# bdaiinstitute/judo

Measured on AMD Instinct MI355X. Metric: rollouts/sec + plan-step ms, leap_cube MPPI 65536xH64, higher is better.
Workload: dtype f32

## Files before the change

### judo_amd/csrc/jh_api.hip

```cpp
#include <algorithm>
#include <cmath>
#include <cstdlib>
#include <cstring>

#include "jh_internal.h"
#include "jh_update_dev.h"

static thread_local char g_err[512] = "";

void jh_set_error(const char* fmt, ...) {
  va_list ap;
  va_start(ap, fmt);
  vsnprintf(g_err, sizeof(g_err), fmt, ap);
  va_end(ap);
}

extern "C" const char* jh_last_error(void) { return g_err; }
extern "C" int jh_version(void) { return 100; }

static int image_cylinders(const jh_blob_header& h, const float* F, const int* I) {
  constexpr int HEADER = 24, BODY_I = 6, BODY_F = 32, BLOCK_I = 4, DOF_F = 20, ACT_I = 2, ACT_F = 8, GEOM_I = 2, GEOM_F = 20, GF_RBOUND = 15;
  if (h.nint < (uint32_t)HEADER || h.nfloat < (uint32_t)HEADER) return 0;
  const long NM = I[0], NBLK = I[1], nv = I[2], nu = I[4], NG = I[5];
  if (NM < 0 || NBLK < 0 || nv < 0 || nu < 0 || NG < 0) return 0;
// ... 279 lines not shown
  const char* e = getenv("JUDO_AMD_LATENCY_SHIFT");
  if (e && e[0] >= '0' && e[0] <= '2') return (e[0] - '0') < most ? (e[0] - '0') : most;
  const long alone = (long)cus * 4;
  for (int sh = most; sh > 0; sh--) if (((long)N << sh) <= alone * rpw) return sh;
  return 0;
}

static int max_fused_knots(const jh_model* m, int H) {
  const bool coop = m->kernel_gen >= 2 && (m->kind == JH_TASK_LEAP_CUBE || m->kind == JH_TASK_FR3_PICK);
  int k = JH_MAX_KNOT_DIM / (m->nu > 0 ? m->nu : 1);
  if (coop && m->kind == JH_TASK_LEAP_CUBE && m->kernel_gen >= 3) return k;
  if (coop) return k < 8 ? k : 8;
  const int lds_k = (m->kind == JH_TASK_CARTPOLE || m->kind == JH_TASK_CYLINDER_PUSH) ? jh_simple_max_knots(m, H) : (g_xcheck.max_knots ? g_xcheck.max_knots(m, H) : 0);
  return k < lds_k ? k : lds_k;
}

extern "C" int jh_model_limits(const jh_model* m, int* out) {
  JH_REQUIRE(m && out, "model_limits: null pointer");
  out[0] = max_fused_knots(m, 1);
  out[1] = JH_MAX_KNOT_DIM;
  out[2] = JH_MAX_ELITES;
  const jh_engine_build* eb = engine_build(m);
  out[3] = eb ? eb->contact_capacity : (articulated(m) ? 32 : 0);
  return JH_OK;
}

extern "C" int jh_model_max_fused_knots(const jh_model* m, int H) {
  JH_REQUIRE(m != nullptr && H >= 1, "model_max_fused_knots: null model or H < 1");
  return max_fused_knots(m, H);
}

extern "C" int jh_model_one_launch_max_knots(const jh_model* m, int H) {
  JH_REQUIRE(m != nullptr && H >= 1, "model_one_launch_max_knots: null model or H < 1");
  const int k = JH_MAX_KNOT_DIM / (m->nu > 0 ? m->nu : 1), lds_k = jh_simple_one_launch_max_knots(m, H);
  return k < lds_k ? k : lds_k;
}

extern "C" int jh_model_set_plan_step_launches(jh_model* m, int launches) {
  JH_REQUIRE(m != nullptr && launches >= 0 && launches <= 2, "model_set_plan_step_launches: launches must be 0 (automatic), 1 or 2");
  JH_REQUIRE(launches != 1 || m->kind == JH_TASK_CARTPOLE || m->kind == JH_TASK_CYLINDER_PUSH, "model_set_plan_step_launches: only the closed-form models have a one-launch plan step");
  m->plan_step_launches = launches;
  return JH_OK;
}

extern "C" int jh_model_set_rollout_schedule(jh_model* m, int mode) {
  JH_REQUIRE(m != nullptr && mode >= 0 && mode <= 2, "model_set_rollout_schedule: mode must be 0 (automatic), 1 (static grid) or 2 (persistent waves wherever the kernel has them)");
  m->rollout_schedule = mode;
  return JH_OK;
}

extern "C" int jh_model_set_rollout_slices(jh_model* m, int slices, int max_workgroups, int flags) {
  JH_REQUIRE(m != nullptr && slices >= 0 && slices <= 64, "model_set_rollout_slices: slices must be 0 (automatic) or 1 .. 64");
  JH_REQUIRE(max_workgroups >= 0, "model_set_rollout_slices: max_workgroups must be 0 (the resident slots) or a positive cap on the queue's grid");
  JH_REQUIRE((flags & ~1) == 0, "model_set_rollout_slices: flags has bit 0 (every hand-off counts as missed) and no other");
  m->rollout_slices = slices; m->rollout_max_workgroups = max_workgroups; m->rollout_slice_flags = flags;
  m->rollout_nbounds = 0;
  return JH_OK;
}

extern "C" int jh_model_set_rollout_slice_bounds(jh_model* m, const int* first_steps, int n) {
  JH_REQUIRE(m != nullptr && n >= 0 && n <= JH_MAX_SLICE_BOUNDS && (n == 0 || first_steps != nullptr), "model_set_rollout_slice_bounds: 0 (none) to %d first steps", JH_MAX_SLICE_BOUNDS);
  for (int i = 0; i < n; i++)
    JH_REQUIRE(first_steps[i] > (i ? first_steps[i - 1] : 0), "model_set_rollout_slice_bounds: first steps must be positive and strictly increasing (entry %d is %d)", i, first_steps[i]);
  for (int i = 0; i < n; i++) m->rollout_bounds[i] = first_steps[i];
  m->rollout_nbounds = n;
  if (n > 0) m->rollout_slices = 0;
  return JH_OK;
}

extern "C" int jh_model_last_rollout_slice_bounds(const jh_model* m, int* out, int cap) {
  JH_REQUIRE(m != nullptr && cap >= 0 && (cap == 0 || out != nullptr), "model_last_rollout_slice_bounds: null model or output");
  const int n = __atomic_load_n(&m->last_rollout_nbounds, __ATOMIC_RELAXED);
  for (int i = 0; i < n && i < cap; i++) out[i] = __atomic_load_n(&m->last_rollout_bounds[i], __ATOMIC_RELAXED);
  return n;
}

void jh_model_note_slice_bounds(const jh_model* m, int slices, int H, const int* bounds) {
  const int n = slices > 1 ? (slices - 1 < 63 ? slices - 1 : 63) : 0;
  for (int i = 0; i < n; i++) __atomic_store_n(&m->last_rollout_bounds[i], bounds ? bounds[i] : (i + 1) * H / slices, __ATOMIC_RELAXED);
  __atomic_store_n(&m->last_rollout_nbounds, n, __ATOMIC_RELAXED);
}

#ifndef JH_AUTO_TAPER
#define JH_AUTO_TAPER 1
#endif
constexpr int JH_TAPER_DEPTH = 4, JH_TAPER_MIN_H = 32;
extern "C" int jh_rollout_slice_schedule(int H, int groups, int wave_slots, int* first_steps, int cap) {
  JH_REQUIRE(H >= 0 && groups >= 0 && wave_slots >= 0 && cap >= 0 && (cap == 0 || first_steps != nullptr), "rollout_slice_schedule: negative argument or null output");
  int b[4], n = 0;
  if (wave_slots > 0 && (long long)groups >= 2ll * wave_slots) {
    if (JH_AUTO_TAPER && H >= JH_TAPER_MIN_H && (long long)groups >= (long long)JH_TAPER_DEPTH * wave_slots) {
      const long long num[4] = {6, 10, 13, 15};
      for (n = 0; n < 4; n++) b[n] = (int)(num[n] * H / 16);
    } else {
      const int S = H < 4 ? H : 4;
      for (int i = 1; i < S; i++) b[n++] = i * H / S;
    }
  }
  for (int i = 0; i < n && i < cap; i++) first_steps[i] = b[i];
  return n;
}

extern "C" int jh_model_last_rollout_slices(const jh_model* m) {
  JH_REQUIRE(m != nullptr, "model_last_rollout_slices: null model");
  return __atomic_load_n(&m->last_rollout_slices, __ATOMIC_RELAXED);
}

extern "C" int jh_model_recomputed_units(jh_model* m) {
  JH_REQUIRE(m != nullptr, "model_recomputed_units: null model");
  int v = 0;
  JH_HIP(hipMemcpy(&v, m->d_stats + JH_STAT_RECOMPUTED, sizeof(int), hipMemcpyDeviceToHost));
  return v;
}

extern "C" int jh_upload_async(void* dst, const void* src, size_t nbytes, void* stream) {
  JH_REQUIRE(dst && src, "upload_async: null pointer");
  JH_HIP(hipMemcpyAsync(dst, src, nbytes, hipMemcpyHostToDevice, (hipStream_t)stream));
  return JH_OK;
}

extern "C" int jh_download_wait(void* dst, const void* src, size_t nbytes, void* stream) {
  JH_REQUIRE(dst && src, "download_wait: null pointer");
  JH_HIP(hipMemcpyAsync(dst, src, nbytes, hipMemcpyDeviceToHost, (hipStream_t)stream));
  JH_HIP(hipStreamSynchronize((hipStream_t)stream));
  return JH_OK;
}

// ... 473 lines not shown
```

### judo_amd/csrc/jh_engine_v5.hip

```cpp
#include <cstddef>
#include <type_traits>

#include "jh_coop.h"

using namespace jh_eng;
using namespace jh_coop;

namespace {

#ifdef JH_V5_WAVESTAMP
__device__ unsigned long long* g_wavestamp = nullptr;
__device__ int g_wavestamp_cap = 0;
#endif

constexpr int G = 16, RPW = 4, WAVE = 64;
constexpr int NCH = 4, NLK = 4;

constexpr int LSMAX = 16;
constexpr int WAVES_PER_EU = 2;
constexpr int WAVES_PER_BLOCK = 4;
constexpr int BFS = 33;
constexpr int PAS = 9;
constexpr int RSPAD = 4;
constexpr int C3PAD = 278;
constexpr int NSLDS = 3;
constexpr double BIGPROB = 0.999999;
constexpr int CVX_STOP_NM = 1000;
#define OPAQUE(x) asm volatile("" : "+v"(x))
constexpr int PARK_F = 5 * 64;
struct SliceBounds { unsigned w[8]; };
constexpr int MAX_BOUND_SLICES = 16;
#define PARK_LD(p) __hip_atomic_load((p), __ATOMIC_RELAXED, __HIP_MEMORY_SCOPE_AGENT)
#define PARK_ST(p, v) __hip_atomic_store((p), (v), __ATOMIC_RELAXED, __HIP_MEMORY_SCOPE_AGENT)
#define WSYNC() do { __builtin_amdgcn_fence(__ATOMIC_RELEASE, "wavefront"); __builtin_amdgcn_wave_barrier(); __builtin_amdgcn_fence(__ATOMIC_ACQUIRE, "wavefront"); } while (0)
#ifndef JH_V5_NSLOT
#define JH_V5_NSLOT 2
#endif
#ifndef JH_V5_NSBIG
#define JH_V5_NSBIG 3
#endif
#ifndef JH_V5_CYL
#define JH_V5_CYL 0
#endif
constexpr int GCYL = 5;
constexpr int NSLOT = JH_V5_NSLOT;
constexpr int NSBIG = JH_V5_NSBIG;
constexpr int NCP = 16 * (NSBIG < NSLDS ? NSBIG : NSLDS);
constexpr int NCAP = 16 * NSBIG;
constexpr int NOVF = NCAP - NCP;
constexpr int MAXHIT = 64;
constexpr int POOL_F = 10;
constexpr int MAXG = 80, MAXLG = 8;
constexpr int CUBE = 17;
constexpr int HITPAIR = 1 << 15;
static_assert(MAXG <= 128, "hand geom pairs are packed into 14 bits");
constexpr int MAXBP = 128;
constexpr int PT_SLOT = JH_PT_SLOT, PT_MAX = JH_PT_MAX, PT_I = JH_PT_I;
constexpr int MAXBPL = 96;
constexpr int NDH = 22 * 23 / 2;
constexpr int NV = 22, NQ = 23, NU = 16, NS = 31, NS_CALTECH = 23, NX = 45, NMB = 17;
constexpr int NBC = 20;
__device__ __forceinline__ bool static_code(int b) { return b == 0 || b >= NMB; }

enum { LC_DAMP = 0, LC_KVD, LC_KP, LC_KV, LC_CLO, LC_CHI, LC_CLIM, LC_FL, LC_FB, LC_FD, LC_INVW, LC_LIMITED, LC_LO, LC_HI, LC_LK, LC_LB, LC_SI, LC_IMCK = LC_SI + 5, LC_N = 25 };

struct __attribute__((aligned(16))) RS {
  float pa[NMB][PAS];
  float xR[NMB][9];
  float qv[NV], g[NV], p[NV], ws[NV];
  float acn[6];
  float Mbb[NCH][10];
  float rhs6[6];
  float cmd[4];
  union {
    struct {
      float bs[NBC][4];
      unsigned short hits[MAXHIT];
      unsigned char bpl[MAXBPL];
    };
    struct { float pk_q[G], pk_fs[G], pk_cq[4], pk_acc; };
  };
  union {
// ... 209 lines not shown
  for (int i = 3; i >= 0; i--) { float s = x[i];
#pragma unroll
    for (int k = i + 1; k < 4; k++) s -= L[tri(k, i)] * x[k];
    x[i] = s * inv[i]; }
}
__device__ __forceinline__ float sel4(const float* a, int j) { return j == 0 ? a[0] : (j == 1 ? a[1] : (j == 2 ? a[2] : a[3])); }

__device__ __forceinline__ float sel4o(const float* a, int j) {
  float lo = (j & 1) ? a[1] : a[0], hi = (j & 1) ? a[3] : a[2];
  asm volatile("" : "+v"(lo), "+v"(hi));
  float r = (j & 2) ? hi : lo;
  asm volatile("" : "+v"(r));
  return r;
}

__device__ __forceinline__ int pidx(int a, int b) { return a * (7 - a) / 2 + (b - a - 1); }
__device__ __forceinline__ bool chain_elim_order(int cmask, int c, int& level, int& parent, int& maxlev) {
  int adj[NCH] = {0, 0, 0, 0};
#pragma unroll
  for (int a = 0; a < NCH; a++)
#pragma unroll
    for (int b = a + 1; b < NCH; b++) if ((cmask >> (4 * a + b)) & 1) { adj[a] |= 1 << b; adj[b] |= 1 << a; }
  int rem = 0xF; bool ok = true;
  level = 0; parent = -1; maxlev = 0;
#pragma unroll
  for (int st = 0; st < NCH; st++) {
    int elig = 0, pr[NCH] = {-1, -1, -1, -1};
#pragma unroll
    for (int a = 0; a < NCH; a++) if ((rem >> a) & 1) {
      const int nbm = adj[a] & rem, deg = __popc(nbm);
      if (deg == 0) elig |= 1 << a;
      else if (deg == 1) {
        const int nb = __ffs(nbm) - 1;
        const int anb = nb == 0 ? adj[0] : (nb == 1 ? adj[1] : (nb == 2 ? adj[2] : adj[3]));
        if (__popc(anb & rem) > 1 || a < nb) { elig |= 1 << a; pr[a] = nb; }
      }
    }
    if (rem != 0 && elig == 0) ok = false;
    if (elig != 0) maxlev = st;
#pragma unroll
    for (int a = 0; a < NCH; a++) if (((elig >> a) & 1) && a == c) { level = st; parent = pr[a]; }
    rem &= ~elig;
  }
  return ok;
}

template <bool MATERIALIZE, int WPB, bool SELF, bool PERSIST = false, bool BATCH = false>
__global__ __launch_bounds__(WAVE * WPB, WAVES_PER_EU) void k_leap_v5(const float* __restrict__ gF, const int* __restrict__ gI, const float* __restrict__ x0, int x0_batched,
                                                   const float* __restrict__ nominal, const float* __restrict__ noise, int ldn,
                                                   const float* __restrict__ sigma, const float* __restrict__ W, const float* __restrict__ lohi,
                                                   const float* __restrict__ tp, int N, int n_offset, int H, int K, float* __restrict__ costs,
                                                   float* __restrict__ knots_out, const float* __restrict__ controls, float* __restrict__ states,
                                                   float* __restrict__ sensors, int* __restrict__ stats_, int dshift_, float* __restrict__ trace, float* __restrict__ ovf_all_, unsigned* __restrict__ head,
                                                   long long batch_blk, long long batch_noise, long long batch_image, unsigned* pflags, int slices_, SliceBounds sb_) {
  static_assert(!BATCH || (!MATERIALIZE && !PERSIST), "batched launches are fused launches on the static grid");
  if constexpr (BATCH) {
    const long long pb = blockIdx.y;
    x0 += pb * batch_blk; nominal += pb * batch_blk; sigma += pb * batch_blk; lohi += pb * batch_blk; tp += pb * batch_blk;
    noise += pb * batch_noise; costs += pb * N; gF += pb * batch_image;
    if (trace) trace += pb * N * H * 15;
    if (NOVF > 0 && ovf_all_) ovf_all_ += pb * N * (NOVF * POOL_F);
  }
  __shared__ RS sRS[RPW * WPB];
  __shared__ float sBody[16 * BFS];
  __shared__ float sTp[16];
  __shared__ float sGeomF[MAXG * GEOM_F];
  __shared__ int sGeomI[MAXG * GEOM_I];
  __shared__ int sLaneG[16 * MAXLG];
  __shared__ float sLane[16 * LC_N];
  __shared__ int sBP[SELF ? 2 * MAXBP : 4];
  __shared__ int sBG[SELF ? 2 * NBC : 4];
  __shared__ float sBB[SELF ? NBC * 8 : 4];
  __shared__ int sGrp[WPB];
  __shared__ int sUnit[4 * WPB];
  const int dshift = PERSIST ? 0 : dshift_;
#ifdef JH_V5_WAVESTAMP
  const unsigned long long ws_entry = wall_clock64(); unsigned long long ws_staged = ws_entry;
#endif
  const int tid = threadIdx.x, wv = tid >> 6, lane = tid & 63, r = lane >> 4;
  int l = lane & 15, c = l >> 2, s = l & 3;
  RS& S = sRS[wv * RPW + r];
  const int nmI = gI[0], nblkI = gI[1], nuI = gI[4], ngI = gI[5], nsiteI = gI[6], nsI = gI[7], oRef = gI[18];
  const int oBodyF = HEADER_F, oDofF = oBodyF + nmI * BODY_F, oActF = oDofF + gI[2] * DOF_F, oGeomF = oActF + nuI * ACT_F, oSiteF = oGeomF + ngI * GEOM_F;
  const int oGeomI = HEADER_I + nmI * BODY_I + nblkI * BLOCK_I + nuI * ACT_I, oSiteI = oGeomI + ngI * GEOM_I;
  const int oLane = gI[11], lgm = gI[12];
  const int oBP = gI[15], oBS = gI[16], nBP = gI[17], oBG = oBP + 2 * nBP;
  for (int i = tid; i < 16 * BODY_F; i += WAVE * WPB) sBody[(i / BODY_F) * BFS + i % BODY_F] = gF[oBodyF + BODY_F + i];
  for (int i = tid; i < ngI * GEOM_F; i += WAVE * WPB) sGeomF[i] = gF[oGeomF + i];
  for (int i = tid; i < ngI * GEOM_I; i += WAVE * WPB) sGeomI[i] = gI[oGeomI + i];
  for (int i = tid; i < 16 * lgm; i += WAVE * WPB) sLaneG[i] = gI[oLane + i];
  if (!MATERIALIZE && tid < 9) sTp[tid] = tp[tid];
  if constexpr (SELF) {
    for (int i = tid; i < 2 * nBP && i < 2 * MAXBP; i += WAVE * WPB) sBP[i] = gI[oBP + i];
    for (int i = tid; i < 2 * NBC; i += WAVE * WPB) sBG[i] = gI[oBG + i];
    for (int i = tid; i < NBC * 8; i += WAVE * WPB) sBB[i] = gF[oBS + i];
  }
  if (tid < 16) {
    const float* df = gF + oDofF + (6 + l) * DOF_F; const float* af = gF + oActF + l * ACT_F;
    float* lc = sLane + l * LC_N;
    lc[LC_DAMP] = df[DF_DAMP]; lc[LC_KVD] = df[DF_KV]; lc[LC_FL] = df[DF_FL]; lc[LC_FB] = df[DF_FB]; lc[LC_FD] = df[DF_FD]; lc[LC_INVW] = df[DF_INVW];
    lc[LC_LIMITED] = df[DF_LIMITED]; lc[LC_LO] = df[DF_LO]; lc[LC_HI] = df[DF_HI]; lc[LC_LK] = df[DF_LK]; lc[LC_LB] = df[DF_LB];
    for (int k = 0; k < 5; k++) lc[LC_SI + k] = df[DF_SOLIMP + k];
    lc[LC_KP] = af[AF_KP]; lc[LC_KV] = af[AF_KV]; lc[LC_CLIM] = af[AF_CLIM]; lc[LC_CLO] = af[AF_CLO]; lc[LC_CHI] = af[AF_CHI];
    lc[LC_IMCK] = l < 6 ? 1.f / (l < 3 ? gF[HF_CMASS] : gF[HF_CINERTIA + (l < 3 ? 0 : l - 3)]) : 0.f;
  }
  const float* lc = sLane + l * LC_N;
  int grp = blockIdx.x * WPB + wv;
  const int ngroups = (N + RPW - 1) / RPW;
  if constexpr (PERSIST) {
    __syncthreads();
#ifdef JH_V5_WAVESTAMP
    ws_staged = wall_clock64();
#endif
  }
  int unit = grp;
  const int nsl = PERSIST ? max(1, min(slices_ & 0xff, H)) : 1, nunits = nsl * ngroups;
  float* park = (float*)(pflags + ((nunits + 3) & ~3));
  bool again = false;
  float q, qd, qc[7], vc[6], acc;
#ifdef JH_V5_WAVESTAMP
  unsigned long long ws_start = 0;
#endif
  for (; !PERSIST || unit < nunits;) {
  bool resumed = false, prefix = false; int hh0 = 0;
  if constexpr (PERSIST) if (again) {
    unit = __builtin_amdgcn_readfirstlane(sUnit[4 * wv + 3]); grp = unit % ngroups; hh0 = __builtin_amdgcn_readfirstlane(sUnit[4 * wv + 1]);
    const int h1 = __builtin_amdgcn_readfirstlane(sUnit[4 * wv + 2]);
    WSYNC();
    if (lane == 0) sUnit[4 * wv] = h1;
  }
  if constexpr (PERSIST) if (!again) {
    grp = unit % ngroups;
    const int sl = unit / ngroups; int h0 = sl * H / nsl, h1 = (sl + 1) * H / nsl;
    if (slices_ & 0x200) {
      const auto bound = [&](int i) -> int { return (int)((sb_.w[i >> 1] >> ((i & 1) << 4)) & 0xffffu); };
      h1 = bound(sl); h0 = sl > 0 ? bound(sl - 1) : 0;
    }
    if (sl > 0) {
      unsigned f = 0;
      if (lane == 0 && !(slices_ & 0x100)) f = __hip_atomic_load(pflags + (unit - ngroups), __ATOMIC_ACQUIRE, __HIP_MEMORY_SCOPE_AGENT);
      resumed = __builtin_amdgcn_readfirstlane(f) != 0;
      if (resumed) { __builtin_amdgcn_fence(__ATOMIC_ACQUIRE, "agent"); hh0 = h0; }
      prefix = !resumed;
    }
    if (lane == 0) { sGrp[wv] = grp; sUnit[4 * wv] = (sl == 0 || resumed) ? h1 : h0; sUnit[4 * wv + 1] = h0; sUnit[4 * wv + 2] = h1; sUnit[4 * wv + 3] = unit; }
  }
#ifdef JH_V5_WAVESTAMP
  if (!PERSIST || !again) ws_start = wall_clock64();
#endif
  const int n = (grp << (2 - dshift)) + (r >> dshift);
  const bool live = n < N && (r & ((1 << dshift) - 1)) == 0;
  const int nc = n < N ? n : N - 1;
  int* stats = stats_; float* ovf_all = ovf_all_;
  if constexpr (PERSIST) if (prefix) {
    stats = nullptr;
    if (NOVF > 0 && ovf_all_) ovf_all = ovf_all_ + ((long long)N + (long long)(blockIdx.x * WPB + wv) * RPW + r - nc) * (NOVF * POOL_F);
  }
  const float h = gF[HF_DT], impratio = gF[HF_IMPRATIO], tol = gF[HF_TOL], lstol = gF[HF_LSTOL]; const int cap = (int)gF[HF_MAXITER];
  const float grav[3] = {gF[HF_GRAV], gF[HF_GRAV + 1], gF[HF_GRAV + 2]};
  const float cmass = gF[HF_CMASS], cI[3] = {gF[HF_CINERTIA], gF[HF_CINERTIA + 1], gF[HF_CINERTIA + 2]};
  const float chs[3] = {gF[HF_CSIZE], gF[HF_CSIZE + 1], gF[HF_CSIZE + 2]}, crb = gF[HF_CRBOUND], ctran = gF[HF_CTRAN];
  const float cK = gF[HF_CK], cB = gF[HF_CB];
  float csi[5]; for (int k = 0; k < 5; k++) csi[k] = gF[HF_SOLIMP + k];
  const float mck = (l < 3 ? cmass : (l == 3 ? cI[0] : (l == 4 ? cI[1] : (l == 5 ? cI[2] : 0.f))));
  if (!PERSIST || !again) {
    const float* xi = x0 + ((MATERIALIZE && x0_batched) ? (size_t)nc * NX : 0);
    for (int k = 0; k < 7; k++) qc[k] = xi[k];
    for (int k = 0; k < 6; k++) vc[k] = xi[NQ + k];
    q = xi[7 + l]; qd = xi[NQ + 6 + l];
  }
  auto knot_at = [&](int k, int ll, int ncc) -> float {
    const int i = k * NU + ll;
    float v = nominal[i];
    if (n_offset + ncc != 0) v = fmaf(sigma[i], noise[(size_t)i * ldn + ncc], v);
    return jh_clampf(v, lohi[ll], lohi[NU + ll]);
  };
  if (!MATERIALIZE) {
    if (knots_out && live && (!PERSIST || unit < ngroups)) for (int k = 0; k < K; k++) knots_out[(size_t)(k * NU + l) * ldn + n] = knot_at(k, l, nc);
  }
  if (!PERSIST || !again) { S.ws[6 + l] = 0.f; if (l < 6) S.ws[l] = 0.f; }
  if (l < 4) S.cmd[l] = l == 0 ? cmass : (l == 1 ? cI[0] : (l == 2 ? cI[1] : cI[2]));
  int n_iters = 0, n_maxed = 0, n_wave_iters = 0;
  if (!PERSIST || !again) acc = 0.f;
  if constexpr (PERSIST) if (resumed) {
    float* pk = park + (size_t)(unit - ngroups) * PARK_F; const int r16 = lane & 48;
    q = PARK_LD(pk + lane); qd = PARK_LD(pk + 64 + lane); S.ws[6 + l] = PARK_LD(pk + 128 + lane);
    for (int k = 0; k < 7; k++) qc[k] = PARK_LD(pk + 192 + r16 + k);
    for (int k = 0; k < 6; k++) vc[k] = PARK_LD(pk + 199 + r16 + k);
    acc = PARK_LD(pk + 205 + r16);
    if (l < 6) S.ws[l] = PARK_LD(pk + 256 + lane);
  }
#ifdef JH_V5_TICKS
  long long cyc[16] = {0, 0, 0, 0, 0, 0, 0, 0, 0, 0, 0, 0, 0, 0, 0, 0}, t0 = clock64();
#define V5_TICK(slot) { long long t__ = clock64(); cyc[slot] += t__ - t0; t0 = t__; }
#else
#define V5_TICK(slot)
#endif
#ifdef JH_V5_COUNT
  int cnt_dense = 0, cnt_it = 0, cnt_l2 = 0, cnt_bp = 0, cnt_hh = 0, cnt_cls[4] = {0, 0, 0, 0};
  enum { CB_SPH = 34, CB_SPHMAX, CB_BOXMAX, CB_L1PAIRPASS, CB_L1LISTPASS, CB_TRIPS, CB_BPAIRS, CB_T, CB_COMBOPASS, CB_CUBEBOX, CB_CUBEBOXLANES, CB_MSPH, CB_MBOX, CB_MT, CB_NOSPH, CB_ONEA, CB_ONEB,
         CB_OWNTRIPS, CB_SPHOVER, CB_FEWSPH, CB_TSAFE, CB_TDROP };
#define V5_CADD(k, v) do { if (stats) atomicAdd(stats + (k), (int)(v)); } while (0)
#define V5_CMAX(k, v) do { if (stats) atomicMax(stats + (k), (int)(v)); } while (0)
#endif
  if constexpr (PERSIST) WSYNC();
  else {
    __syncthreads();
#ifdef JH_V5_WAVESTAMP
    ws_staged = wall_clock64();
#endif
  }

  const int hend = PERSIST ? __builtin_amdgcn_readfirstlane(sUnit[4 * wv]) : H;
  for (int hh = hh0; hh < hend; hh++) {
    OPAQUE(l); c = l >> 2; s = l & 3;
    const float* lc = sLane + l * LC_N;
    float u;
    if (MATERIALIZE) u = controls[((size_t)nc * H + hh) * NU + l];
    else {
      u = 0.f;
      {
        int lo_ = lane; OPAQUE(lo_);
        const int g_ = PERSIST ? sGrp[wv] : (int)(blockIdx.x * WPB + wv);
        const int n_ = (g_ << (2 - dshift)) + ((lo_ >> 4) >> dshift), nc_ = n_ < N ? n_ : N - 1;
        for (int k = 0; k < K; k++) u = fmaf(W[hh * K + k], knot_at(k, l, nc_), u);
      }
    }
    float Mrow[NLK], fs_own, a0_own;
    {
      float ax[NLK][3], og[NLK][3], Rown[9], pown[3];
      {
        float nn = rsqrtf(qc[3] * qc[3] + qc[4] * qc[4] + qc[5] * qc[5] + qc[6] * qc[6]);
        qc[3] *= nn; qc[4] *= nn; qc[5] *= nn; qc[6] *= nn;
        float Rc[9]; quat2mat(Rc, qc + 3);
        float P[3] = {0, 0, 0}, R[9] = {1, 0, 0, 0, 1, 0, 0, 0, 1};
        float sn_own, cs_own; sincosf(q, &sn_own, &cs_own);
#pragma unroll
        for (int j = 0; j < NLK; j++) {
          const float* bf = sBody + (4 * c + j) * BFS;
          float P2[3], R0[9];
          if (j == 0) { for (int k = 0; k < 3; k++) P2[k] = bf[BF_LPOS + k]; for (int k = 0; k < 9; k++) R0[k] = bf[BF_LR + k]; }
          else { mulMV(P2, R, bf + BF_LPOS); for (int k = 0; k < 3; k++) P2[k] += P[k]; mulMM(R0, R, bf + BF_LR); }
          const float* al = bf + BF_AXIS;
// ... 1023 lines not shown
      float inv4[4]; chol4(L, inv4); fwd4(L, inv4, x4); bwd4(L, inv4, x4);
      const float qacc = sel4(x4, s);
      qd = fmaf(h, qacc, qd); q = fmaf(h, qd, q);
      WSYNC();
      for (int k = 0; k < 6; k++) vc[k] = S.qv[k];
      for (int k = 0; k < 4; k++) qc[3 + k] = S.pk_cq[k];
      if (!MATERIALIZE) acc = S.pk_acc;
      {
        const float aw[3] = {S.acn[3], S.acn[4], S.acn[5]}; float ab[3]; mulMTV(ab, S.xR[0], aw);
        for (int k = 0; k < 3; k++) { vc[k] = fmaf(h, S.acn[k], vc[k]); vc[3 + k] = fmaf(h, ab[k], vc[3 + k]); }
        if (l < 3) S.ws[3 + l] = l == 0 ? ab[0] : (l == 1 ? ab[1] : ab[2]);
      }
      for (int k = 0; k < 3; k++) qc[k] = fmaf(h, vc[k], qc[k]);
      float wn = sqrtf(vc[3] * vc[3] + vc[4] * vc[4] + vc[5] * vc[5]), ang = wn * h;
      if (ang > 0.f) {
        float sn, cs; sincosf(0.5f * ang, &sn, &cs); float kk = sn / wn;
        float dq[4] = {cs, vc[3] * kk, vc[4] * kk, vc[5] * kk}, *qq = qc + 3;
        float r0 = qq[0] * dq[0] - qq[1] * dq[1] - qq[2] * dq[2] - qq[3] * dq[3];
        float r1 = qq[0] * dq[1] + qq[1] * dq[0] + qq[2] * dq[3] - qq[3] * dq[2];
        float r2 = qq[0] * dq[2] - qq[1] * dq[3] + qq[2] * dq[0] + qq[3] * dq[1];
        float r3 = qq[0] * dq[3] + qq[1] * dq[2] - qq[2] * dq[1] + qq[3] * dq[0];
        qq[0] = r0; qq[1] = r1; qq[2] = r2; qq[3] = r3;
      }
      float nn = rsqrtf(qc[3] * qc[3] + qc[4] * qc[4] + qc[5] * qc[5] + qc[6] * qc[6]);
      qc[3] *= nn; qc[4] *= nn; qc[5] *= nn; qc[6] *= nn;
    }
    V5_TICK(7)
    if (MATERIALIZE) {
      if (states && live) {
        float* o = states + ((size_t)nc * H + hh) * NX;
        o[7 + l] = q; o[NQ + 6 + l] = qd;
        if (l < 7) o[l] = qc[l];
        if (l < 6) o[NQ + l] = vc[l];
      }
    } else acc += leap_step_cost(sTp, qc);
    WSYNC();
  }
  if constexpr (PERSIST) {
    again = __builtin_amdgcn_readfirstlane(sUnit[4 * wv]) < __builtin_amdgcn_readfirstlane(sUnit[4 * wv + 2]);
    if (again) { if (lane == 0 && stats_) atomicAdd(stats_ + JH_STAT_RECOMPUTED, 1); continue; }
  }
  int usteps = H; bool last = true;
  if constexpr (PERSIST) { const int h0 = __builtin_amdgcn_readfirstlane(sUnit[4 * wv + 1]), h1 = __builtin_amdgcn_readfirstlane(sUnit[4 * wv + 2]); usteps = h1 - h0; last = h1 >= H; unit = __builtin_amdgcn_readfirstlane(sUnit[4 * wv + 3]); }
#ifdef JH_V5_COUNT
  if (stats) { if (lane == 0) { atomicAdd(stats + 24, cnt_dense); atomicAdd(stats + 25, cnt_it); atomicAdd(stats + 26, cnt_l2); atomicAdd(stats + 28, usteps); } if (l == 0 && live) { atomicAdd(stats + 27, cnt_bp); atomicAdd(stats + 29, cnt_hh); for (int k = 0; k < 4; k++) atomicAdd(stats + 30 + k, cnt_cls[k]); } }
#endif
#ifdef JH_V5_TICKS
  if (lane == 0 && stats) { for (int k = 0; k < 8; k++) atomicAdd((unsigned long long*)(stats + 4) + k, (unsigned long long)cyc[k]);
                            for (int k = 0; k < 16; k++) atomicAdd((unsigned long long*)(stats + 384) + k, (unsigned long long)cyc[k]); }
#endif
  if (!MATERIALIZE && live && l == 0 && last) costs[n] = acc / (float)H;
  if (stats && live && l == 0) { if (n_maxed) atomicAdd(stats + JH_STAT_ITER_CAP, n_maxed); atomicAdd(stats + JH_STAT_ITERS, n_iters); atomicAdd(stats + JH_STAT_STEPS, usteps); }
  if (stats && lane == 0 && live) { atomicAdd(stats + JH_STAT_WAVE_ITERS, n_wave_iters); atomicAdd(stats + JH_STAT_WAVE_STEPS, usteps); }
  if constexpr (PERSIST) if (!last) {
    float* pk = park + (size_t)unit * PARK_F;
    float pv = l == 13 ? acc : 0.f;
    for (int k = 0; k < 7; k++) if (l == k) pv = qc[k];
    for (int k = 0; k < 6; k++) if (l == 7 + k) pv = vc[k];
    PARK_ST(pk + lane, q); PARK_ST(pk + 64 + lane, qd); PARK_ST(pk + 128 + lane, S.ws[6 + l]); PARK_ST(pk + 192 + lane, pv); PARK_ST(pk + 256 + lane, l < 6 ? S.ws[l] : 0.f);
    __threadfence();
    if (lane == 0) __hip_atomic_store(pflags + unit, 1u, __ATOMIC_RELEASE, __HIP_MEMORY_SCOPE_AGENT);
  }
#ifdef JH_V5_WAVESTAMP
  if (lane == 0 && g_wavestamp && (PERSIST ? unit : grp) < g_wavestamp_cap) {
    unsigned long long* w = g_wavestamp + (size_t)(PERSIST ? unit : grp) * 6;
    w[0] = ((unsigned long long)blockIdx.x << 32) | ((unsigned long long)wv << 8) | (__smid() & 0xff); w[1] = ws_entry; w[2] = ws_staged; w[3] = ws_start; w[4] = wall_clock64(); w[5] = 1;
  }
#endif
  if constexpr (!PERSIST) break;
  else {
    int t = 0;
    if (lane == 0) t = (int)atomicAdd(head, 1u);
    unit = (int)(gridDim.x * WPB) + __builtin_amdgcn_readfirstlane(t);
  }
  }
}

bool model_is_leap(const jh_model* m) {
  return m->kind == JH_TASK_LEAP_CUBE && m->nq == 23 && m->nv == 22 && m->nu == 16 && (m->ns == NS || (m->ns == NS_CALTECH && m->h_i.size() > 18 && m->h_i[18] > 0)) && m->h_i.size() > 17 &&
         m->h_i[0] == 17 && m->h_i[1] == 4 && m->h_i[11] > 0 && m->h_i[5] <= MAXG && m->h_i[12] <= MAXLG && m->h_i[17] <= MAXBP
         && m->h_f.size() > (size_t)HF_CINERTIA + 2 && m->h_f[HF_CINERTIA] == m->h_f[HF_CINERTIA + 1] && m->h_f[HF_CINERTIA] == m->h_f[HF_CINERTIA + 2]
         ;
}

int device_cus(const jh_model* m) {
  int v = 0;
  return (hipDeviceGetAttribute(&v, hipDeviceAttributeMultiprocessorCount, m->device) == hipSuccess && v > 0) ? v : 256;
}

int leap_refusal(const jh_model* m, const char* who) {
  if (!model_is_leap(m)) { if (who) jh_set_error("%s: the cooperative engine kernel is instantiated for leap_cube only", who); return JH_ERR_UNSUPPORTED; }
  if ((m->cylinders > 0) != (JH_V5_CYL != 0)) { if (who) jh_set_error("%s: an image with cylinder geoms runs on the cylinder build of the leap kernel and no other image does (%d cylinders)", who, m->cylinders); return JH_ERR_UNSUPPORTED; }
  return JH_OK;
}
bool accepts(const jh_model* m) { return leap_refusal(m, nullptr) == JH_OK; }

struct LeapArgs {
  const jh_rollout_args& a; const float* gF; const int* gI; int* stats; int dshift, grid;
  int x0_batched = 0; const float* controls = nullptr; float *states = nullptr, *sensors = nullptr;
  float* ovf = nullptr; unsigned *head = nullptr, *pflags = nullptr; int slices = 0; SliceBounds sb = {};
  long long batch_blk = 0, batch_noise = 0, batch_image = 0;
};

LeapArgs leap_args(const jh_model* m, const jh_rollout_args& a, const float* gF, const int* gI, int rollouts) {
  const int dshift = jh_latency_shift(rollouts, RPW), per_block = (RPW >> dshift) * WAVES_PER_BLOCK;
  return {a, gF, gI, m->d_stats, dshift, (a.N + per_block - 1) / per_block};
}

size_t ovf_bytes(size_t rows) { return NOVF > 0 ? rows * NOVF * POOL_F * sizeof(float) : 0; }

template <bool MATERIALIZE, bool SELF, bool PERSIST = false, bool BATCH = false>
void launch(const LeapArgs& k, dim3 grid, hipStream_t st) {
  const jh_rollout_args& a = k.a;
  hipLaunchKernelGGL((k_leap_v5<MATERIALIZE, WAVES_PER_BLOCK, SELF, PERSIST, BATCH>), grid, dim3(WAVE * WAVES_PER_BLOCK), 0, st, k.gF, k.gI, a.x0, k.x0_batched, a.nominal, a.noise, a.ldn,
                     a.sigma, a.W, a.lohi, a.tp, a.N, a.n_offset, a.H, a.K, a.costs, a.knots_out, k.controls, k.states, k.sensors, k.stats, k.dshift, a.trace, k.ovf, k.head,
                     k.batch_blk, k.batch_noise, k.batch_image, k.pflags, k.slices, k.sb);
}

bool hand_contacts(const jh_model* m) { return m->self_collision && m->h_i[17] > 0; }

}

#ifndef JH_V5_NAME
#define JH_V5_NAME(f) f
#endif
#ifdef JH_V5_WAVESTAMP
extern "C" int JH_V5_NAME(jh_v5_wavestamp_buffer)(unsigned long long* buf, int groups) {
  JH_HIP(hipMemcpyToSymbol(HIP_SYMBOL(g_wavestamp), &buf, sizeof(buf)));
  JH_HIP(hipMemcpyToSymbol(HIP_SYMBOL(g_wavestamp_cap), &groups, sizeof(groups)));
  return JH_OK;
}
#endif
static int rollout_cost(const jh_model* m, const jh_rollout_args& a, hipStream_t st) {
  if (int rc = leap_refusal(m, "rollout_cost")) return rc;
  const int N = a.N, H = a.H;
  LeapArgs k = leap_args(m, a, m->d_f, m->d_i, N);
  bool persist = k.dshift == 0 && m->rollout_schedule != 1; int slots = 0;
  if (persist) { slots = 2 * device_cus(m); persist = m->rollout_schedule == 2 || k.grid > slots; }
  const int ngroups = (N + RPW - 1) / RPW;
  int slices = 1, bounds[JH_MAX_SLICE_BOUNDS], nb = 0; bool table = false;
  if (persist) {
    if (m->rollout_nbounds > 0) { for (int i = 0; i < m->rollout_nbounds; i++) if (m->rollout_bounds[i] < H) bounds[nb++] = m->rollout_bounds[i]; slices = nb + 1; }
    else if (m->rollout_slices > 0) slices = m->rollout_slices;
    else { nb = jh_rollout_slice_schedule(H, ngroups, slots * WAVES_PER_BLOCK, bounds, JH_MAX_SLICE_BOUNDS); slices = nb + 1; }
    if (slices > H) slices = H;
    if (slices < 1 || (long long)slices * ngroups > 0x7fffffffll) slices = 1;
    for (int i = 0; i < nb && slices == nb + 1; i++) table = table || bounds[i] != (i + 1) * H / slices;
    if (table && (slices > MAX_BOUND_SLICES || H > 0xffff)) { slices = 1; table = false; }
  }
  int qgrid = k.grid;
  if (persist) { if (qgrid > slots) qgrid = slots; if (m->rollout_max_workgroups > 0 && qgrid > m->rollout_max_workgroups) qgrid = m->rollout_max_workgroups; }
  size_t flag_words = 0, queue_bytes = 0, ovf_b = 0;
  float* scratch = nullptr; unsigned* head = nullptr;
  for (;;) {
    flag_words = slices > 1 ? (((size_t)slices * ngroups + 3) & ~(size_t)3) : 0;
    const size_t park_floats = slices > 1 ? (size_t)(slices - 1) * ngroups * PARK_F : 0, own_rows = slices > 1 ? (size_t)qgrid * WAVES_PER_BLOCK * RPW : 0;
    queue_bytes = persist ? 16 + (flag_words + park_floats) * sizeof(float) : 0;
    ovf_b = ovf_bytes((size_t)N + own_rows);
    if (ovf_b > 0 || persist) scratch = jh_launch_scratch(m, ovf_b + queue_bytes, st, ovf_b > 0 && slices == 1);
    if (scratch || slices == 1) break;
    slices = 1; table = false;
  }
  if (scratch && persist && hipMemsetAsync(scratch, 0, 16 + flag_words * sizeof(unsigned), st) != hipSuccess) { (void)hipGetLastError(); persist = false; }
  if (!scratch) persist = false;
  if (persist) { head = (unsigned*)scratch; k.grid = qgrid; } else { slices = 1; table = false; }
  if (table) for (int i = 0; i < MAX_BOUND_SLICES; i++) k.sb.w[i >> 1] |= (unsigned)(i < nb ? bounds[i] : H) << ((i & 1) << 4);
  jh_model_note_slice_bounds(m, slices, H, table ? bounds : nullptr);
  if (scratch && ovf_b > 0) k.ovf = scratch + (head ? queue_bytes / sizeof(float) : 0);
  __atomic_store_n(&m->last_rollout_slices, persist ? slices : 0, __ATOMIC_RELAXED);
  k.head = head; k.pflags = head ? head + 4 : nullptr; k.slices = slices | ((m->rollout_slice_flags & 1) << 8) | (table ? 0x200 : 0);
  if (hand_contacts(m)) { if (persist) launch<false, true, true>(k, dim3(k.grid), st); else launch<false, true, false>(k, dim3(k.grid), st); }
  else { if (persist) launch<false, false, true>(k, dim3(k.grid), st); else launch<false, false, false>(k, dim3(k.grid), st); }
  return jh_launch_done(scratch, st);
}

static int materialize(const jh_model* m, const float* x0, int x0_batched, const float* controls, int N, int H, float* states, float* sensors, hipStream_t st) {
  if (int rc = leap_refusal(m, "rollout_materialize")) return rc;
  jh_rollout_args a = {};
  a.x0 = x0; a.N = N; a.H = H;
  LeapArgs k = leap_args(m, a, m->d_f, m->d_i, N);
  k.x0_batched = x0_batched; k.controls = controls; k.states = states; k.sensors = sensors;
  if (const size_t b = ovf_bytes(N)) k.ovf = jh_launch_scratch(m, b, st);
  if (hand_contacts(m)) launch<true, true>(k, dim3(k.grid), st);
  else launch<true, false>(k, dim3(k.grid), st);
  return jh_launch_done(k.ovf, st);
}

static int rollout_cost_batch(const jh_model* m, const jh_rollout_args& a, const jh_rollout_batch& s, hipStream_t st) {
  if (int rc = leap_refusal(m, "plan_step_batch")) return rc;
  JH_REQUIRE((long long)s.B * a.N <= 0x7fffffffll, "plan_step_batch: B * N = %lld rollouts exceed one launch", (long long)s.B * a.N);
  LeapArgs k = leap_args(m, a, s.images, s.ints, s.B * a.N);
  k.batch_blk = s.blk_stride; k.batch_noise = s.noise_stride; k.batch_image = s.image_stride;
  if (const size_t b = ovf_bytes((size_t)s.B * a.N)) k.ovf = jh_launch_scratch(m, b, st);
  if (hand_contacts(m)) launch<false, true, false, true>(k, dim3(k.grid, s.B), st);
  else launch<false, false, false, true>(k, dim3(k.grid, s.B), st);
  return jh_launch_done(k.ovf, st);
}

#ifndef __HIP_DEVICE_COMPILE__
const jh_engine_build JH_V5_NAME(jh_engine5_build) = {JH_V5_CYL ? "leap, cylinders" : NCAP > 48 ? "leap, 64 contacts" : "leap, 48 contacts", accepts, rollout_cost, rollout_cost_batch, materialize, NCAP};
#endif
```

### judo_amd/csrc/jh_internal.h

```cpp
#pragma once

#include <hip/hip_runtime.h>

#include <cstdarg>
#include <cstdint>
#include <cstdio>
#include <vector>

#include "judo_amd.h"
#include "judo_amd_xcheck.h"

#define JH_BLOB_MAGIC 0x314D484Au
#define JH_BLOB_VERSION 1u
#define JH_NSTATS 512
constexpr int JH_PT_SLOT = 19, JH_PT_MAX = 4, JH_PT_I = 9, JH_PT_LEN = 1 + JH_PT_MAX * JH_PT_I;

struct jh_blob_header {
  uint32_t magic, version, kind, nq, nv, nu, ns, ntaskparam, nfloat, nint;
  uint32_t reserved[6];
};

constexpr int JH_MAX_SLICE_BOUNDS = 15;

struct jh_model {
  int device, kind, nq, nv, nu, ns, ntaskparam;
  size_t nf, ni;
  float* d_f;
  int* d_i;
  int kernel_gen;
  int contact_capacity;
  int cylinders;
  int arm_pairs;
  int self_collision;
  int rollout_schedule;
  int rollout_slices = 0, rollout_max_workgroups = 0, rollout_slice_flags = 0;
  int rollout_bounds[JH_MAX_SLICE_BOUNDS] = {}, rollout_nbounds = 0;
  mutable int last_rollout_bounds[63] = {}, last_rollout_nbounds = 0;
  mutable int last_rollout_slices = 0;
  int plan_step_launches;
  mutable int one_launch_steps = 0;
  mutable int ovf_fallbacks = 0;
  int* d_stats;
  std::vector<float> h_f;
  std::vector<int> h_i;
};

void jh_set_error(const char* fmt, ...);
void jh_model_note_slice_bounds(const jh_model* m, int slices, int H, const int* bounds);

inline float* jh_launch_scratch(const jh_model* m, size_t bytes, hipStream_t st, bool overflow_rows = true) {
  hipMemPool_t pool = nullptr; void* p = nullptr;
  if (hipDeviceGetDefaultMemPool(&pool, m->device) == hipSuccess && pool && hipMallocFromPoolAsync(&p, bytes, pool, st) == hipSuccess) return (float*)p;
  (void)hipGetLastError();
  if (!overflow_rows) return nullptr;
  if (__atomic_fetch_add(&m->ovf_fallbacks, 1, __ATOMIC_RELAXED) == 0)
    fprintf(stderr, "judo_amd: no stream-ordered scratch for the contacts above the LDS pool (%zu bytes): this launch runs with the LDS capacity alone; see jh_model_stats out[6]\n", bytes);
  return nullptr;
}

#define JH_HIP(call)                                                                      \
  do {                                                                                    \
    hipError_t e__ = (call);                                                              \
    if (e__ != hipSuccess) {                                                              \
      jh_set_error("%s failed: %s (%s:%d)", #call, hipGetErrorString(e__), __FILE__, __LINE__); \
      return JH_ERR_HIP;                                                                  \
    }                                                                                     \
  } while (0)

inline int jh_launch_done(float* ovf, hipStream_t st) {
  const hipError_t e = hipGetLastError();
  const hipError_t f = ovf ? hipFreeAsync(ovf, st) : hipSuccess;
  if (e != hipSuccess) { jh_set_error("kernel launch failed: %s", hipGetErrorString(e)); return JH_ERR_HIP; }
  if (f != hipSuccess) { jh_set_error("hipFreeAsync failed: %s", hipGetErrorString(f)); return JH_ERR_HIP; }
  return JH_OK;
}

#define JH_REQUIRE(cond, ...)    \
  do {                           \
    if (!(cond)) {               \
      jh_set_error(__VA_ARGS__); \
      return JH_ERR_INVALID;     \
    }                            \
  } while (0)

enum {
  CP_DT = 0, CP_G, CP_MCART, CP_MPOLE, CP_L, CP_IPOLE, CP_DAMP_X, CP_DAMP_TH, CP_KP, CP_KV, CP_CTRL_LO, CP_CTRL_HI, CP_CTRL_LIMITED,
  CP_FRC_LO, CP_FRC_HI, CP_FRC_LIMITED, CP_X_LO, CP_X_HI, CP_X_LIMITED, CP_LIM_K, CP_LIM_B, CP_SOLIMP0, CP_SOLIMP1, CP_SOLIMP2,
  CP_SOLIMP3, CP_SOLIMP4, CP_INVW_X, CP_TIP, CP_NPARAM
};
enum {
  CY_DT = 0, CY_MP, CY_MC, CY_DAMP_P, CY_DAMP_C, CY_KP, CY_KV, CY_CTRL_LO, CY_CTRL_HI, CY_CTRL_LIMITED, CY_FRC_LO, CY_FRC_HI,
  CY_FRC_LIMITED, CY_RSUM, CY_CON_K, CY_CON_B, CY_SOLIMP0, CY_SOLIMP1, CY_SOLIMP2, CY_SOLIMP3, CY_SOLIMP4, CY_TRAN, CY_MU, CY_SITE_Z,
  CY_MARGIN, CY_NPARAM
};

struct jh_rollout_args {
  const float *x0, *nominal, *noise; int ldn;
  const float *sigma, *W, *lohi, *tp; int phase, N, n_offset, H, K;
  float *costs, *knots_out, *trace;
};
struct jh_rollout_batch {
// ... 64 lines not shown
```

Baseline: 1.365 million.

## Replace park flags with nonce-tagged park words for slice hand-off

Persistent slice hand-off used to write the parked state, issue a threadfence, and then release a per-unit flag, and the consumer acquired that flag before reading the parked rows. Each parked float is now stored as a 64-bit word whose high half is a hash tag built from a per-launch nonce, the unit and the row. The consumer loads the rows and treats them as valid only when every tag matches, which removes the fence, the flag release/acquire and the per-launch memset of the flag array. In exchange the park buffer doubles in size, the consumer always loads all five rows before deciding, and a stale word that happens to match its tag could be accepted. Two test flags are added: one parks a torn row and one parks nothing.

```diff
diff --git a/judo_amd/csrc/jh_api.hip b/judo_amd/csrc/jh_api.hip
--- a/judo_amd/csrc/jh_api.hip
+++ b/judo_amd/csrc/jh_api.hip
@@ -355,7 +355,7 @@
 extern "C" int jh_model_set_rollout_slices(jh_model* m, int slices, int max_workgroups, int flags) {
   JH_REQUIRE(m != nullptr && slices >= 0 && slices <= 64, "model_set_rollout_slices: slices must be 0 (automatic) or 1 .. 64");
   JH_REQUIRE(max_workgroups >= 0, "model_set_rollout_slices: max_workgroups must be 0 (the resident slots) or a positive cap on the queue's grid");
-  JH_REQUIRE((flags & ~1) == 0, "model_set_rollout_slices: flags has bit 0 (every hand-off counts as missed) and no other");
+  JH_REQUIRE((flags & ~0xd) == 0, "model_set_rollout_slices: flags has bit 0 (every hand-off counts as missed), bit 2 (producers park a torn row) and bit 3 (producers park nothing) and no other");
   m->rollout_slices = slices; m->rollout_max_workgroups = max_workgroups; m->rollout_slice_flags = flags;
   m->rollout_nbounds = 0;
   return JH_OK;
@@ -376,6 +376,13 @@
   const int n = __atomic_load_n(&m->last_rollout_nbounds, __ATOMIC_RELAXED);
   for (int i = 0; i < n && i < cap; i++) out[i] = __atomic_load_n(&m->last_rollout_bounds[i], __ATOMIC_RELAXED);
   return n;
+}
+
+unsigned jh_launch_nonce() {
+  static unsigned counter = 0;
+  unsigned v;
+  do v = __atomic_add_fetch(&counter, 1u, __ATOMIC_RELAXED); while (v == 0);
+  return v;
 }
 
 void jh_model_note_slice_bounds(const jh_model* m, int slices, int H, const int* bounds) {
diff --git a/judo_amd/csrc/jh_engine_v5.hip b/judo_amd/csrc/jh_engine_v5.hip
--- a/judo_amd/csrc/jh_engine_v5.hip
+++ b/judo_amd/csrc/jh_engine_v5.hip
@@ -28,6 +28,12 @@
 constexpr int CVX_STOP_NM = 1000;
 #define OPAQUE(x) asm volatile("" : "+v"(x))
 constexpr int PARK_F = 5 * 64;
+__device__ __forceinline__ unsigned park_tag(unsigned nonce, int ticket, int row) {
+  unsigned x = (unsigned)ticket * (unsigned)PARK_F + (unsigned)row;
+  x ^= x >> 16; x *= 0x85ebca6bu; x ^= x >> 13; x *= 0xc2b2ae35u; x ^= x >> 16;
+  const unsigned t = nonce ^ x;
+  return t ? t : 1u;
+}
 struct SliceBounds { unsigned w[8]; };
 constexpr int MAX_BOUND_SLICES = 16;
 #define PARK_LD(p) __hip_atomic_load((p), __ATOMIC_RELAXED, __HIP_MEMORY_SCOPE_AGENT)
@@ -343,7 +349,7 @@
                                                    const float* __restrict__ tp, int N, int n_offset, int H, int K, float* __restrict__ costs,
                                                    float* __restrict__ knots_out, const float* __restrict__ controls, float* __restrict__ states,
                                                    float* __restrict__ sensors, int* __restrict__ stats_, int dshift_, float* __restrict__ trace, float* __restrict__ ovf_all_, unsigned* __restrict__ head,
-                                                   long long batch_blk, long long batch_noise, long long batch_image, unsigned* pflags, int slices_, SliceBounds sb_) {
+                                                   long long batch_blk, long long batch_noise, long long batch_image, unsigned long long* park, int slices_, SliceBounds sb_, unsigned nonce_) {
   static_assert(!BATCH || (!MATERIALIZE && !PERSIST), "batched launches are fused launches on the static grid");
   if constexpr (BATCH) {
     const long long pb = blockIdx.y;
@@ -406,13 +412,13 @@
   }
   int unit = grp;
   const int nsl = PERSIST ? max(1, min(slices_ & 0xff, H)) : 1, nunits = nsl * ngroups;
-  float* park = (float*)(pflags + ((nunits + 3) & ~3));
   bool again = false;
   float q, qd, qc[7], vc[6], acc;
 #ifdef JH_V5_WAVESTAMP
   unsigned long long ws_start = 0;
 #endif
   for (; !PERSIST || unit < nunits;) {
+  float pw[5] = {0.f, 0.f, 0.f, 0.f, 0.f};
   bool resumed = false, prefix = false; int hh0 = 0;
   if constexpr (PERSIST) if (again) {
     unit = __builtin_amdgcn_readfirstlane(sUnit[4 * wv + 3]); grp = unit % ngroups; hh0 = __builtin_amdgcn_readfirstlane(sUnit[4 * wv + 1]);
@@ -428,10 +434,13 @@
       h1 = bound(sl); h0 = sl > 0 ? bound(sl - 1) : 0;
     }
     if (sl > 0) {
-      unsigned f = 0;
-      if (lane == 0 && !(slices_ & 0x100)) f = __hip_atomic_load(pflags + (unit - ngroups), __ATOMIC_ACQUIRE, __HIP_MEMORY_SCOPE_AGENT);
-      resumed = __builtin_amdgcn_readfirstlane(f) != 0;
-      if (resumed) { __builtin_amdgcn_fence(__ATOMIC_ACQUIRE, "agent"); hh0 = h0; }
+      if (!(slices_ & 0x100)) {
+        const int pu = unit - ngroups; unsigned long long* pk = park + (size_t)pu * PARK_F; unsigned long long w[5]; unsigned bad = 0;
+        for (int k = 0; k < 5; k++) w[k] = PARK_LD(pk + 64 * k + lane);
+        for (int k = 0; k < 5; k++) { bad |= (unsigned)(w[k] >> 32) ^ park_tag(nonce_, pu, 64 * k + lane); pw[k] = __uint_as_float((unsigned)w[k]); }
+        resumed = __all(bad == 0);
+      }
+      if (resumed) hh0 = h0;
       prefix = !resumed;
     }
     if (lane == 0) { sGrp[wv] = grp; sUnit[4 * wv] = (sl == 0 || resumed) ? h1 : h0; sUnit[4 * wv + 1] = h0; sUnit[4 * wv + 2] = h1; sUnit[4 * wv + 3] = unit; }
@@ -474,12 +483,11 @@
   int n_iters = 0, n_maxed = 0, n_wave_iters = 0;
   if (!PERSIST || !again) acc = 0.f;
   if constexpr (PERSIST) if (resumed) {
-    float* pk = park + (size_t)(unit - ngroups) * PARK_F; const int r16 = lane & 48;
-    q = PARK_LD(pk + lane); qd = PARK_LD(pk + 64 + lane); S.ws[6 + l] = PARK_LD(pk + 128 + lane);
-    for (int k = 0; k < 7; k++) qc[k] = PARK_LD(pk + 192 + r16 + k);
-    for (int k = 0; k < 6; k++) vc[k] = PARK_LD(pk + 199 + r16 + k);
-    acc = PARK_LD(pk + 205 + r16);
-    if (l < 6) S.ws[l] = PARK_LD(pk + 256 + lane);
+    q = pw[0]; qd = pw[1]; S.ws[6 + l] = pw[2];
+    for (int k = 0; k < 7; k++) qc[k] = __shfl(pw[3], k, 16);
+    for (int k = 0; k < 6; k++) vc[k] = __shfl(pw[3], 7 + k, 16);
+    acc = __shfl(pw[3], 13, 16);
+    if (l < 6) S.ws[l] = pw[4];
   }
 #ifdef JH_V5_TICKS
   long long cyc[16] = {0, 0, 0, 0, 0, 0, 0, 0, 0, 0, 0, 0, 0, 0, 0, 0}, t0 = clock64();
@@ -1609,14 +1617,15 @@
   if (!MATERIALIZE && live && l == 0 && last) costs[n] = acc / (float)H;
   if (stats && live && l == 0) { if (n_maxed) atomicAdd(stats + JH_STAT_ITER_CAP, n_maxed); atomicAdd(stats + JH_STAT_ITERS, n_iters); atomicAdd(stats + JH_STAT_STEPS, usteps); }
   if (stats && lane == 0 && live) { atomicAdd(stats + JH_STAT_WAVE_ITERS, n_wave_iters); atomicAdd(stats + JH_STAT_WAVE_STEPS, usteps); }
-  if constexpr (PERSIST) if (!last) {
-    float* pk = park + (size_t)unit * PARK_F;
+  if constexpr (PERSIST) if (!last && !(slices_ & 0x800)) {
+    unsigned long long* pk = park + (size_t)unit * PARK_F;
     float pv = l == 13 ? acc : 0.f;
     for (int k = 0; k < 7; k++) if (l == k) pv = qc[k];
     for (int k = 0; k < 6; k++) if (l == 7 + k) pv = vc[k];
-    PARK_ST(pk + lane, q); PARK_ST(pk + 64 + lane, qd); PARK_ST(pk + 128 + lane, S.ws[6 + l]); PARK_ST(pk + 192 + lane, pv); PARK_ST(pk + 256 + lane, l < 6 ? S.ws[l] : 0.f);
-    __threadfence();
-    if (lane == 0) __hip_atomic_store(pflags + unit, 1u, __ATOMIC_RELEASE, __HIP_MEMORY_SCOPE_AGENT);
+    const float out[5] = {q, qd, S.ws[6 + l], pv, l < 6 ? S.ws[l] : 0.f};
+    const int rows = (slices_ & 0x400) ? 3 : 5;
+    for (int k = 0; k < 5; k++)
+      if (k < rows) PARK_ST(pk + 64 * k + lane, ((unsigned long long)park_tag(nonce_, unit, 64 * k + lane) << 32) | __float_as_uint(out[k]));
   }
 #ifdef JH_V5_WAVESTAMP
   if (lane == 0 && g_wavestamp && (PERSIST ? unit : grp) < g_wavestamp_cap) {
@@ -1655,7 +1664,7 @@
 struct LeapArgs {
   const jh_rollout_args& a; const float* gF; const int* gI; int* stats; int dshift, grid;
   int x0_batched = 0; const float* controls = nullptr; float *states = nullptr, *sensors = nullptr;
-  float* ovf = nullptr; unsigned *head = nullptr, *pflags = nullptr; int slices = 0; SliceBounds sb = {};
+  float* ovf = nullptr; unsigned* head = nullptr; unsigned long long* park = nullptr; int slices = 0; SliceBounds sb = {}; unsigned nonce = 0;
   long long batch_blk = 0, batch_noise = 0, batch_image = 0;
 };
 
@@ -1671,7 +1680,7 @@
   const jh_rollout_args& a = k.a;
   hipLaunchKernelGGL((k_leap_v5<MATERIALIZE, WAVES_PER_BLOCK, SELF, PERSIST, BATCH>), grid, dim3(WAVE * WAVES_PER_BLOCK), 0, st, k.gF, k.gI, a.x0, k.x0_batched, a.nominal, a.noise, a.ldn,
                      a.sigma, a.W, a.lohi, a.tp, a.N, a.n_offset, a.H, a.K, a.costs, a.knots_out, k.controls, k.states, k.sensors, k.stats, k.dshift, a.trace, k.ovf, k.head,
-                     k.batch_blk, k.batch_noise, k.batch_image, k.pflags, k.slices, k.sb);
+                     k.batch_blk, k.batch_noise, k.batch_image, k.park, k.slices, k.sb, k.nonce);
 }
 
 bool hand_contacts(const jh_model* m) { return m->self_collision && m->h_i[17] > 0; }
@@ -1707,25 +1716,25 @@
   }
   int qgrid = k.grid;
   if (persist) { if (qgrid > slots) qgrid = slots; if (m->rollout_max_workgroups > 0 && qgrid > m->rollout_max_workgroups) qgrid = m->rollout_max_workgroups; }
-  size_t flag_words = 0, queue_bytes = 0, ovf_b = 0;
+  size_t queue_bytes = 0, ovf_b = 0;
   float* scratch = nullptr; unsigned* head = nullptr;
   for (;;) {
-    flag_words = slices > 1 ? (((size_t)slices * ngroups + 3) & ~(size_t)3) : 0;
-    const size_t park_floats = slices > 1 ? (size_t)(slices - 1) * ngroups * PARK_F : 0, own_rows = slices > 1 ? (size_t)qgrid * WAVES_PER_BLOCK * RPW : 0;
-    queue_bytes = persist ? 16 + (flag_words + park_floats) * sizeof(float) : 0;
+    const size_t park_words = slices > 1 ? (size_t)(slices - 1) * ngroups * PARK_F : 0, own_rows = slices > 1 ? (size_t)qgrid * WAVES_PER_BLOCK * RPW : 0;
+    queue_bytes = persist ? 16 + park_words * sizeof(unsigned long long) : 0;
     ovf_b = ovf_bytes((size_t)N + own_rows);
     if (ovf_b > 0 || persist) scratch = jh_launch_scratch(m, ovf_b + queue_bytes, st, ovf_b > 0 && slices == 1);
     if (scratch || slices == 1) break;
     slices = 1; table = false;
   }
-  if (scratch && persist && hipMemsetAsync(scratch, 0, 16 + flag_words * sizeof(unsigned), st) != hipSuccess) { (void)hipGetLastError(); persist = false; }
+  if (scratch && persist && hipMemsetAsync(scratch, 0, 16, st) != hipSuccess) { (void)hipGetLastError(); persist = false; }
   if (!scratch) persist = false;
   if (persist) { head = (unsigned*)scratch; k.grid = qgrid; } else { slices = 1; table = false; }
   if (table) for (int i = 0; i < MAX_BOUND_SLICES; i++) k.sb.w[i >> 1] |= (unsigned)(i < nb ? bounds[i] : H) << ((i & 1) << 4);
   jh_model_note_slice_bounds(m, slices, H, table ? bounds : nullptr);
   if (scratch && ovf_b > 0) k.ovf = scratch + (head ? queue_bytes / sizeof(float) : 0);
   __atomic_store_n(&m->last_rollout_slices, persist ? slices : 0, __ATOMIC_RELAXED);
-  k.head = head; k.pflags = head ? head + 4 : nullptr; k.slices = slices | ((m->rollout_slice_flags & 1) << 8) | (table ? 0x200 : 0);
+  k.head = head; k.park = head ? (unsigned long long*)(head + 4) : nullptr; k.nonce = slices > 1 ? jh_launch_nonce() : 0;
+  k.slices = slices | ((m->rollout_slice_flags & 1) << 8) | (table ? 0x200 : 0) | ((m->rollout_slice_flags & 0xc) << 8);
   if (hand_contacts(m)) { if (persist) launch<false, true, true>(k, dim3(k.grid), st); else launch<false, true, false>(k, dim3(k.grid), st); }
   else { if (persist) launch<false, false, true>(k, dim3(k.grid), st); else launch<false, false, false>(k, dim3(k.grid), st); }
   return jh_launch_done(scratch, st);
diff --git a/judo_amd/csrc/jh_internal.h b/judo_amd/csrc/jh_internal.h
--- a/judo_amd/csrc/jh_internal.h
+++ b/judo_amd/csrc/jh_internal.h
@@ -47,6 +47,7 @@
 
 void jh_set_error(const char* fmt, ...);
 void jh_model_note_slice_bounds(const jh_model* m, int slices, int H, const int* bounds);
+unsigned jh_launch_nonce();
 
 inline float* jh_launch_scratch(const jh_model* m, size_t bytes, hipStream_t st, bool overflow_rows = true) {
   hipMemPool_t pool = nullptr; void* p = nullptr;
```

New measurement: 1.377 million, median of 6. No clear change (+0.8%).
